# qinjr/SCoRe

Measured on AMD Instinct MI355X. Metric: train samples/sec @ batch=1024, higher is better.
Workload: dtype f32

## Files before the change

### score_amd/csrc/common.h

```cpp
#pragma once
#include <hip/hip_runtime.h>
#include <stdint.h>
#include "../../include/score_hip.h"

#define SCORE_WAVE 64

#if (defined(X3_PROBE_NOLOADA) || defined(X3_PROBE_NOLOADB) || defined(X3_PROBE_NOSPLIT) || defined(X3_PROBE_NOLDSW) ||      \
     defined(X3_PROBE_NOLDSR) || defined(X3_PROBE_NOMFMA) || defined(X3_PROBE_NOSTORE) || defined(PANEL_PROBE_NOMFMA) ||      \
     defined(PANEL_PROBE_NOALOAD) || defined(PANEL_PROBE_NOASTORE) || defined(PANEL_PROBE_NOBLOAD) ||                         \
     defined(PANEL_PROBE_NOREAD) || defined(PANEL_PROBE_NOCSTORE) || defined(GRP_NOMFMA) || defined(GRP_NOSTORE) ||           \
     defined(GRP_NOXLOAD) || defined(GSP_NOMFMA) || defined(GSP_NOBLOAD) || defined(GSP_NOSTORE) || defined(GSP_NOXLOAD) ||   \
     defined(XGP_NOMFMA) || defined(XGP_NOSTORE) || defined(XGP_NOXLOAD) || defined(AFP_NOPRELOAD) || defined(AFP_NOMFMA) ||  \
     defined(AFP_NOEPI) || defined(AFP_NOBUILD) || defined(AFP_NOTAIL) || defined(AFP_NOINP)) &&                              \
    !defined(SCORE_PROBE_BUILD)
#error "a wrong-by-design probe switch needs -DSCORE_PROBE_BUILD (tools/*_probe.py pass it; score_amd/build.py never does)"
#endif

#define SCORE_CHECK_LAUNCH()                      \
  do {                                            \
    hipError_t e__ = hipGetLastError();           \
    if (e__ != hipSuccess) return (int)e__;       \
  } while (0)

#define SCORE_TRY(expr)                           \
  do {                                            \
    int rc__ = (expr);                            \
    if (rc__ != 0) return rc__;                   \
  } while (0)

static inline int64_t cdiv64(int64_t a, int64_t b) { return (a + b - 1) / b; }
static inline int64_t align_up64(int64_t a, int64_t b) { return cdiv64(a, b) * b; }

__device__ __forceinline__ float4 ld4(const float* p) { return *reinterpret_cast<const float4*>(p); }
__device__ __forceinline__ void st4(float* p, float4 v) { *reinterpret_cast<float4*>(p) = v; }
typedef float score_v4f __attribute__((ext_vector_type(4)));
__device__ __forceinline__ float4 ld4_global(const float* p) {
  const score_v4f v = *(const __attribute__((address_space(1))) score_v4f*)p;
  return make_float4(v.x, v.y, v.z, v.w);
}
__device__ __forceinline__ float ld1_global(const float* p) { return *(const __attribute__((address_space(1))) float*)p; }
__device__ __forceinline__ float dot4(float4 a, float4 b) {
  return fmaf(a.w, b.w, fmaf(a.z, b.z, fmaf(a.y, b.y, a.x * b.x)));
}
__device__ __forceinline__ float4 fma4(float s, float4 a, float4 acc) {
  acc.x = fmaf(s, a.x, acc.x); acc.y = fmaf(s, a.y, acc.y);
  acc.z = fmaf(s, a.z, acc.z); acc.w = fmaf(s, a.w, acc.w);
  return acc;
}
__device__ __forceinline__ float4 add4(float4 a, float4 b) {
  return make_float4(a.x + b.x, a.y + b.y, a.z + b.z, a.w + b.w);
}
__device__ __forceinline__ void score_adam1(float& p, float& m, float& v, float g, float omb1, float omb2, float alpha,
                                            float eps) {
  m = __builtin_fmaf(g - m, omb1, m);
  v = __builtin_fmaf(__builtin_fmaf(g, g, -v), omb2, v);
#if defined(SCORE_ADAM_IEEE_DIV)
  p = p - (m * alpha) / (sqrtf(v) + eps);
#else
  p = p - (m * alpha) * __builtin_amdgcn_rcpf(__builtin_amdgcn_sqrtf(v) + eps);
#endif
}
__device__ __forceinline__ void score_adam_dense_body(float* __restrict__ p, float* __restrict__ m, float* __restrict__ v,
                                                      const float* __restrict__ g, int64_t n4, int64_t n, int64_t n_reg, float l2,
                                                      float alpha, float omb1, float omb2, float eps, int blk, int nblk) {
  int64_t i = (int64_t)blk * blockDim.x + threadIdx.x;
  const int64_t stride = (int64_t)nblk * blockDim.x;
  for (; i < n4; i += stride) {
    float4 mm = ld4(m + i * 4), vv = ld4(v + i * 4), gg = ld4(g + i * 4);
    int64_t e = i * 4;
    if (e >= n_reg && gg.x == 0.f && gg.y == 0.f && gg.z == 0.f && gg.w == 0.f && mm.x == 0.f && mm.y == 0.f &&
        mm.z == 0.f && mm.w == 0.f && vv.x == 0.f && vv.y == 0.f && vv.z == 0.f && vv.w == 0.f)
      continue;
    float4 pp = ld4(p + i * 4);
    if (e < n_reg) {
      gg.x = e + 0 < n_reg ? fmaf(l2, pp.x, gg.x) : gg.x;
      gg.y = e + 1 < n_reg ? fmaf(l2, pp.y, gg.y) : gg.y;
      gg.z = e + 2 < n_reg ? fmaf(l2, pp.z, gg.z) : gg.z;
      gg.w = e + 3 < n_reg ? fmaf(l2, pp.w, gg.w) : gg.w;
    }
    score_adam1(pp.x, mm.x, vv.x, gg.x, omb1, omb2, alpha, eps);
    score_adam1(pp.y, mm.y, vv.y, gg.y, omb1, omb2, alpha, eps);
    score_adam1(pp.z, mm.z, vv.z, gg.z, omb1, omb2, alpha, eps);
    score_adam1(pp.w, mm.w, vv.w, gg.w, omb1, omb2, alpha, eps);
    st4(p + i * 4, pp); st4(m + i * 4, mm); st4(v + i * 4, vv);
  }
  if (blk == 0 && threadIdx.x < (unsigned)(n - n4 * 4)) {
    int64_t e = n4 * 4 + threadIdx.x;
    float pp = p[e], mm = m[e], vv = v[e], gg = g[e];
    if (e < n_reg) gg = fmaf(l2, pp, gg);
    score_adam1(pp, mm, vv, gg, omb1, omb2, alpha, eps);
    p[e] = pp; m[e] = mm; v[e] = vv;
  }
}
__device__ __forceinline__ float sigmoidf_(float x) { return 1.0f / (1.0f + expf(-x)); }

__device__ __forceinline__ float group_sum(float v, int gs) {
  for (int off = gs >> 1; off > 0; off >>= 1) v += __shfl_xor(v, off, SCORE_WAVE);
  return v;
}
__device__ __forceinline__ float wave_sum(float v) { return group_sum(v, SCORE_WAVE); }

template <int CTRL>
__device__ __forceinline__ float dpp_f32(float v) {
  return __int_as_float(__builtin_amdgcn_update_dpp(0, __float_as_int(v), CTRL, 0xF, 0xF, true));
}
template <int N>
__device__ __forceinline__ void group_sum_n(float (&v)[N], int gs) {
  if (gs >= 2) {
#pragma unroll
    for (int n = 0; n < N; ++n) v[n] += dpp_f32<0xB1>(v[n]);
  }
  if (gs >= 4) {
#pragma unroll
    for (int n = 0; n < N; ++n) v[n] += dpp_f32<0x4E>(v[n]);
  }
  if (gs >= 8) {
#pragma unroll
    for (int n = 0; n < N; ++n) v[n] += dpp_f32<0x141>(v[n]);
  }
  if (gs >= 16) {
#pragma unroll
    for (int n = 0; n < N; ++n) v[n] += dpp_f32<0x140>(v[n]);
  }
  if (gs >= 32) {
    const int lane = (int)__builtin_amdgcn_mbcnt_hi(~0u, __builtin_amdgcn_mbcnt_lo(~0u, 0u));
    const int a16 = (lane ^ 16) << 2, a32 = (lane ^ 32) << 2;
    float t[N];
#pragma unroll
    for (int n = 0; n < N; ++n) t[n] = __int_as_float(__builtin_amdgcn_ds_bpermute(a16, __float_as_int(v[n])));
#pragma unroll
    for (int n = 0; n < N; ++n) v[n] += t[n];
    if (gs >= 64) {
#pragma unroll
      for (int n = 0; n < N; ++n) t[n] = __int_as_float(__builtin_amdgcn_ds_bpermute(a32, __float_as_int(v[n])));
#pragma unroll
      for (int n = 0; n < N; ++n) v[n] += t[n];
    }
  }
}
__device__ __forceinline__ float wave_max(float v) {
  for (int off = 32; off > 0; off >>= 1) v = fmaxf(v, __shfl_xor(v, off, SCORE_WAVE));
  return v;
}

__device__ __forceinline__ void xcd_tile_coords_n(int nwg, int orig, int gx, int gy, int& bx, int& by, int& bz) {
  const int q = nwg >> 3, r = nwg & 7, xcd = orig & 7;
  const int wg = (xcd < r ? xcd * (q + 1) : r * (q + 1) + (xcd - r) * q) + (orig >> 3);
  bx = wg % gx;
  const int t = wg / gx;
  by = t % gy;
  bz = t / gy;
}
__device__ __forceinline__ void xcd_tile_coords(int gx, int gy, int& bx, int& by, int& bz) {
  xcd_tile_coords_n((int)gridDim.x, (int)blockIdx.x, gx, gy, bx, by, bz);
}

__device__ __forceinline__ float hash_uniform(uint64_t seed, uint64_t idx) {
  uint64_t z = seed + 0x9E3779B97F4A7C15ull * (idx + 1);
  z = (z ^ (z >> 30)) * 0xBF58476D1CE4E5B9ull;
  z = (z ^ (z >> 27)) * 0x94D049BB133111EBull;
  z = z ^ (z >> 31);
  return (float)(z >> 40) * (1.0f / 16777216.0f);
}
```

### score_amd/csrc/head_fused.hip

```cpp
#include "common.h"
#include "kernels.h"

typedef float hf_f32x4 __attribute__((ext_vector_type(4)));

namespace {

constexpr int HF_ROWS = 16;
constexpr int HF_NW = 8;
constexpr int HF_CH = 16;

template <int NT>
__device__ __forceinline__ void hf_tiles(hf_f32x4 (&acc)[NT], const float* __restrict__ xs, int LD, int Kp, int K,
                                         const float* __restrict__ W, int ldw, const int (&n0)[NT], int N, int lc, int lq) {
  const int KQ = Kp >> 2;
  const int kbase = lq * KQ;
  int col[NT];
  bool cok[NT];
#pragma unroll
  for (int t = 0; t < NT; ++t) {
    cok[t] = n0[t] >= 0 && n0[t] + lc < N;
    col[t] = cok[t] ? n0[t] + lc : 0;
  }
  float b0[NT][HF_CH], b1[NT][HF_CH];
  auto fetch = [&](float (&bb)[NT][HF_CH], int s0) {
// ... 125 lines not shown
      hf_f32x4 acc[1] = {{0.f, 0.f, 0.f, 0.f}};
      const int t0 = tb + wave;
      const int n0[1] = {t0 < tend ? t0 * 16 : -1};
      if (n0[0] >= 0) hf_tiles<1>(acc, xs, LD0, Kp0, Dh, a.W1, N1, n0, N1, lc, lq);
      const int col = n0[0] + lc;
      const float bias = a.b1[min(max(col, 0), N1 - 1)];
      if (n0[0] >= 0 && col < N1) {
#pragma unroll
        for (int r = 0; r < 4; ++r) {
          const int row = b0 + lq * 4 + r;
          const float v = hf_act(acc[0][r], bias, a.drop, a.keep, a.mask0, seed0, row, col, N1);
          if (row < a.B) a.f1[(int64_t)row * N1 + col] = v;
        }
      }
    }
    return;
  }
  if (phase == 2) {
    for (int e = tid; e < HF_ROWS * N1; e += 64 * HF_NW) {
      const int i = e / N1, j = e - i * N1;
      const int row = min(b0 + i, a.B - 1);
      f1s[i * LD1 + j] = a.f1[(int64_t)row * N1 + j];
    }
  }
  for (int tb = 0; phase == 0 && tb < nt1; tb += 2 * HF_NW) {
    hf_f32x4 acc[2] = {{0.f, 0.f, 0.f, 0.f}, {0.f, 0.f, 0.f, 0.f}};
    const int t0 = tb + wave, t1 = tb + HF_NW + wave;
    const int n0[2] = {t0 < nt1 ? t0 * 16 : -1, t1 < nt1 ? t1 * 16 : -1};
    if (n0[0] >= 0) hf_tiles<2>(acc, xs, LD0, Kp0, Dh, a.W1, N1, n0, N1, lc, lq);
    float bias1[2];
#pragma unroll
    for (int t = 0; t < 2; ++t) bias1[t] = a.b1[min(max(n0[t] + lc, 0), N1 - 1)];
#pragma unroll
    for (int t = 0; t < 2; ++t) {
      const int col = n0[t] + lc;
      if (n0[t] < 0 || col >= N1) continue;
      const float bias = bias1[t];
#pragma unroll
      for (int r = 0; r < 4; ++r) {
        const int i = lq * 4 + r, row = b0 + i;
        const float v = hf_act(acc[t][r], bias, a.drop, a.keep, a.mask0, seed0, row, col, N1);
        f1s[i * LD1 + col] = v;
        if (row < a.B) a.f1[(int64_t)row * N1 + col] = v;
      }
    }
  }
  __syncthreads();

  const int nt2 = (N2 + 15) >> 4;
  for (int tb = 0; tb < nt2; tb += HF_NW) {
    hf_f32x4 acc[1] = {{0.f, 0.f, 0.f, 0.f}};
    const int t0 = tb + wave;
    const int n0[1] = {t0 < nt2 ? t0 * 16 : -1};
    if (n0[0] >= 0) hf_tiles<1>(acc, f1s, LD1, Kp1, N1, a.W2, N2, n0, N2, lc, lq);
    const int col = n0[0] + lc;
    const float bias2 = a.b2[min(max(col, 0), N2 - 1)];
    if (n0[0] >= 0 && col < N2) {
      const float bias = bias2;
#pragma unroll
      for (int r = 0; r < 4; ++r) {
        const int i = lq * 4 + r, row = b0 + i;
        const float v = hf_act(acc[0][r], bias, a.drop, a.keep, a.mask1, seed1, row, col, N2);
        f2s[i * LD2 + col] = v;
        if (row < a.B) a.f2[(int64_t)row * N2 + col] = v;
      }
    }
  }
  __syncthreads();

  if (wave == 0) {
    const int i = lane >> 2, part = lane & 3;
    float s = 0.f;
    for (int n = part; n < N2; n += 4) s = fmaf(f2s[i * LD2 + n], a.W3[n], s);
    s += __shfl_xor(s, 1, 64);
    s += __shfl_xor(s, 2, 64);
    const int row = b0 + i;
    if (part == 0 && row < a.B) {
      const float z = s + a.b3[0];
      const float p = sigmoidf_(z);
      const float lab = (float)a.label[row];
      const float eps = 1e-7f;
      a.logit[row] = z;
      a.y[row] = p;
      a.lossb[row] = -lab * logf(p + eps) - (1.0f - lab) * logf(1.0f - p + eps);
      const float dp = (-lab / (p + eps) + (1.0f - lab) / (1.0f - p + eps)) / (float)a.Bglobal;
      const float dl = dp * p * (1.0f - p);
      a.dlogit[row] = dl;
      xs[i] = dl;
    }
  }
  __syncthreads();
  if (a.dz2) {
    for (int e = tid; e < HF_ROWS * N2; e += 64 * HF_NW) {
      const int i = e / N2, n = e - i * N2, row = b0 + i;
      const float q = xs[i] * a.W3[n] / a.keep;
      if (row < a.B) a.dz2[(int64_t)row * N2 + n] = f2s[i * LD2 + n] > 0.f ? q : 0.f;
    }
  }
}


constexpr int AF_NW = 8;

struct AttnFwdArgs {
  int B, T, H, NI, N1, N2, S;
  const float* q; const float* ur; const float* ir; const float* info;
  const float* Weff; const float* qz;
  const float* W4; const float* b4; const float* w5; const float* b5; const int32_t* length;
  float* inp; float* a1; float* a2; float* score; float* head; int ldh, off_u, off_i;
  int wcopies; int64_t wstride;
};

__device__ __forceinline__ void af_build(const AttnFwdArgs& a, float* __restrict__ xs, int LD, int Kp, int row0,
                                         int row_end, int t0, int nthr) {
  const int Dk = 2 * a.H + a.NI, Dk4 = Dk >> 2, K2 = 2 * Dk;
  const int total = 16 * Dk4;
  constexpr int U = 4;
  for (int e0 = t0; e0 < total; e0 += U * nthr) {
    float4 k[U], qq[U];
    int ii[U], jj[U], gg[U];
    bool ok[U];
#pragma unroll
    for (int u = 0; u < U; ++u) {
      const int e = e0 + u * nthr;
      const int ec = e < total ? e : 0;
      ii[u] = ec / Dk4; jj[u] = (ec - ii[u] * Dk4) * 4;
      gg[u] = row0 + ii[u];
      ok[u] = e < total && gg[u] < row_end;
      const int g = gg[u] < row_end ? gg[u] : row_end - 1;
      const int j = jj[u];
      const float* src = j < a.H ? a.ur + (int64_t)g * a.H + j
                                 : (j < 2 * a.H ? a.ir + (int64_t)g * a.H + (j - a.H) : a.info + (int64_t)g * a.NI + (j - 2 * a.H));
      k[u] = ld4(src);
      qq[u] = ld4(a.q + (int64_t)(g / a.T) * Dk + j);
    }
#pragma unroll
    for (int u = 0; u < U; ++u) {
      if (e0 + u * nthr >= total) continue;
      float4 kk = k[u], qk = make_float4(qq[u].x * kk.x, qq[u].y * kk.y, qq[u].z * kk.z, qq[u].w * kk.w);
      if (ok[u]) {
#ifndef AFP_NOINP
        st4(a.inp + (int64_t)gg[u] * K2 + jj[u], kk);
        st4(a.inp + (int64_t)gg[u] * K2 + Dk + jj[u], qk);
#endif
      } else {
        kk = make_float4(0.f, 0.f, 0.f, 0.f); qk = kk;
      }
      *reinterpret_cast<float4*>(xs + ii[u] * LD + jj[u]) = kk;
      *reinterpret_cast<float4*>(xs + ii[u] * LD + Dk + jj[u]) = qk;
    }
  }
  for (int e = t0; e < 16 * (Kp - K2); e += nthr) {
    const int i = e / (Kp - K2), j = e - i * (Kp - K2);
    xs[i * LD + K2 + j] = 0.f;
  }
}

template <int KQ>
__global__ __launch_bounds__(64 * AF_NW) void attn_fwd_fused_kernel(const AttnFwdArgs a) {
  extern __shared__ float sm[];
  const int T = a.T, H = a.H, N1 = a.N1, N2 = a.N2;
  const int Dk = 2 * H + a.NI, K2 = 2 * Dk, Kp = 4 * KQ, LD = Kp + 4;
  const int L1 = N1 + 1, L2 = N2 + 1;
  float* xs0 = sm;
  float* xs1 = xs0 + 16 * LD;
  float* a1s = xs1 + 16 * LD;
  float* w4s = a1s + a.S * T * L1;
  float* a2s = w4s + N1 * N2;
  float* scs = a2s + a.S * T * L2;
  const int tid = threadIdx.x, lane = tid & 63, wave = tid >> 6;
  const int lc = lane & 15, lq = lane >> 4;
  const int b0 = blockIdx.x * a.S;
  const int ns = min(a.S, a.B - b0);
  const int row0 = b0 * T, row_end = row0 + ns * T;
  const int ntile = (ns * T + 15) >> 4;
  const int ntn = (N1 + 15) >> 4;

  float breg[KQ];
  if (wave < ntn) {
    const int col = wave * 16 + lc;
    const float* Wsrc = a.Weff + (int64_t)((blockIdx.x >> 3) % a.wcopies) * a.wstride;
#pragma unroll
    for (int s_ = 0; s_ < KQ; ++s_) {
      const int k = lq * KQ + s_;
#ifdef AFP_NOPRELOAD
      const float w = (float)(k + col) * 1e-3f;
#else
      const float w = Wsrc[(int64_t)(k < K2 ? k : K2 - 1) * N1 + (col < N1 ? col : N1 - 1)];
#endif
      breg[s_] = w * ((k < K2 && col < N1) ? 1.0f : 0.0f);
    }
  }
  for (int i = tid; i < N1 * N2; i += 64 * AF_NW) w4s[i] = a.W4[i];
  af_build(a, xs0, LD, Kp, row0, row_end, tid, 64 * AF_NW);
  __syncthreads();
  for (int m = 0; m < ntile; ++m) {
    float* xs = (m & 1) ? xs1 : xs0;
    if (wave < ntn) {
      hf_f32x4 acc[1] = {{0.f, 0.f, 0.f, 0.f}};
      const int n0[1] = {wave * 16};
      const float* xrow = xs + lc * LD + lq * KQ;
#ifndef AFP_NOMFMA
#ifdef AFP_TWOACC
      hf_f32x4 acc2 = {0.f, 0.f, 0.f, 0.f};
#pragma unroll
      for (int s4 = 0; s4 < KQ; s4 += 4) {
        const float4 av = *reinterpret_cast<const float4*>(xrow + s4);
        acc[0] = __builtin_amdgcn_mfma_f32_16x16x4f32(av.x, breg[s4 + 0], acc[0], 0, 0, 0);
        acc2 = __builtin_amdgcn_mfma_f32_16x16x4f32(av.y, breg[s4 + 1], acc2, 0, 0, 0);
        acc[0] = __builtin_amdgcn_mfma_f32_16x16x4f32(av.z, breg[s4 + 2], acc[0], 0, 0, 0);
        acc2 = __builtin_amdgcn_mfma_f32_16x16x4f32(av.w, breg[s4 + 3], acc2, 0, 0, 0);
      }
      acc[0] += acc2;
#else
#pragma unroll
      for (int s4 = 0; s4 < KQ; s4 += 4) {
        const float4 av = *reinterpret_cast<const float4*>(xrow + s4);
        acc[0] = __builtin_amdgcn_mfma_f32_16x16x4f32(av.x, breg[s4 + 0], acc[0], 0, 0, 0);
        acc[0] = __builtin_amdgcn_mfma_f32_16x16x4f32(av.y, breg[s4 + 1], acc[0], 0, 0, 0);
        acc[0] = __builtin_amdgcn_mfma_f32_16x16x4f32(av.z, breg[s4 + 2], acc[0], 0, 0, 0);
        acc[0] = __builtin_amdgcn_mfma_f32_16x16x4f32(av.w, breg[s4 + 3], acc[0], 0, 0, 0);
      }
#endif
#else
      acc[0][0] = xrow[0] * breg[0] + breg[KQ - 1];
#endif
      const int col = n0[0] + lc;
      if (col < N1) {
#pragma unroll
        for (int r = 0; r < 4; ++r) {
          const int i = m * 16 + lq * 4 + r;
          const int g = row0 + i;
          if (g < row_end) {
#ifdef AFP_NOEPI
            const float v = fmaxf(acc[0][r], 0.f);
            a1s[i * L1 + col] = v;
#else
            const float v = fmaxf(acc[0][r] + a.qz[(int64_t)(g / T) * N1 + col], 0.f);
            a1s[i * L1 + col] = v;
            a.a1[(int64_t)g * N1 + col] = v;
#endif
          }
        }
      }
    } else if (m + 1 < ntile) {
#ifndef AFP_NOBUILD
      af_build(a, (m & 1) ? xs0 : xs1, LD, Kp, row0 + (m + 1) * 16, row_end, tid - 64 * ntn, 64 * (AF_NW - ntn));
#endif
    }
    __syncthreads();
  }

#ifdef AFP_NOTAIL
  return;
#endif
  const int gsz = 64 * AF_NW / a.S, s_ = tid / gsz, gt = tid - s_ * gsz;
  const bool live = s_ < ns;
  const int b = b0 + (live ? s_ : 0);
  const float* a1b = a1s + s_ * T * L1;
  float* a2l = a2s + s_ * T * L2;
  float* sc = scs + s_ * T;
  if (live) {
    float* a2b = a.a2 + (int64_t)b * T * N2;
    for (int i = gt; i < T * N2; i += gsz) {
      const int t = i / N2, n = i - t * N2;
      float acc = 0.f;
#pragma unroll 8
      for (int k = 0; k < N1; ++k) acc = fmaf(a1b[t * L1 + k], w4s[k * N2 + n], acc);
      const float v = fmaxf(acc + a.b4[n], 0.f);
      a2l[t * L2 + n] = v;
      a2b[i] = v;
    }
  }
  __syncthreads();
  if (live) {
    const int len = a.length[b];
    for (int t = gt; t < T; t += gsz) {
      float acc = 0.f;
      for (int n = 0; n < N2; ++n) acc = fmaf(a2l[t * L2 + n], a.w5[n], acc);
      sc[t] = t < len ? acc + a.b5[0] : -4294967295.0f;
    }
  }
  __syncthreads();
  float mx = -INFINITY, den = 0.f;
  if (live) {
    for (int t = 0; t < T; ++t) mx = fmaxf(mx, sc[t]);
    for (int t = 0; t < T; ++t) den += expf(sc[t] - mx);
  }
  __syncthreads();
  if (live) {
    for (int t = gt; t < T; t += gsz) {
      const float v = expf(sc[t] - mx) / den;
      sc[t] = v;
      a.score[(int64_t)b * T + t] = v;
    }
  }
  __syncthreads();
  if (live) {
    for (int j = gt; j < 2 * H; j += gsz) {
      const bool us = j < H;
      const float* rep = (us ? a.ur : a.ir) + (int64_t)b * T * H + (us ? j : j - H);
      float acc = 0.f;
      for (int t = 0; t < T; ++t) acc = fmaf(rep[(int64_t)t * H], sc[t], acc);
      const int off = us ? a.off_u : a.off_i;
      if (off >= 0) a.head[(int64_t)b * a.ldh + off + (us ? j : j - H)] = acc;
    }
  }
}


constexpr int AB_NTW = 5;
constexpr int AB_KQ = 20;

struct AttnBwdArgs {
  int B, T, H, NI, S;
  const float* da1; const float* Weff; const float* q; const float* ur; const float* ir; const float* info;
  const float* score; const float* dhead; int ldh, off_u, off_i;
  float* dur; float* dir; float* dinfo; float* dq;
  int pool, N2;
  const float* a2; const float* a1; const float* w5; const float* W4; const int32_t* length;
  float* ds; float* da2; float* da1_out;
};

__global__ __launch_bounds__(64 * AF_NW) void attn_inp_bwd_fused_kernel(const AttnBwdArgs a) {
  extern __shared__ float sm[];
  const int T = a.T, H = a.H, NI = a.NI;
  const int Dk = 2 * H + NI, Dk4 = Dk >> 2, K2 = 2 * Dk, N1 = 4 * AB_KQ;
  const int LDA = N1 + 4, LDO = K2 + 4;
  const int RT = ((a.S * T + 15) >> 4) << 4;
  float* da1s = sm;
  float* ot = da1s + RT * LDA;
  float* dqs = ot + 16 * LDO;
  float* sds = dqs + a.S * Dk;
  float* d2s = sds + a.S * T;
  float* w4s = d2s + a.S * T * (a.N2 + 1);
  const int tid = threadIdx.x, lane = tid & 63, wave = tid >> 6;
  const int lc = lane & 15, lq = lane >> 4;
  const int b0 = blockIdx.x * a.S;
  const int ns = min(a.S, a.B - b0);
  const int row0 = b0 * T, row_end = row0 + ns * T;
  const int ntile = (ns * T + 15) >> 4;
  const int ntn = (K2 + 15) >> 4;

  float breg[AB_NTW][AB_KQ];
#pragma unroll
  for (int t = 0; t < AB_NTW; ++t) {
    const int n = (wave + AF_NW * t) * 16 + lc;
    const float msk = n < K2 ? 1.0f : 0.0f;
    const float* wrow = a.Weff + (int64_t)(n < K2 ? n : K2 - 1) * N1 + lq * AB_KQ;
#pragma unroll
    for (int s4 = 0; s4 < AB_KQ; s4 += 4) {
      const float4 w = ld4(wrow + s4);
      breg[t][s4 + 0] = w.x * msk; breg[t][s4 + 1] = w.y * msk; breg[t][s4 + 2] = w.z * msk; breg[t][s4 + 3] = w.w * msk;
    }
  }
  for (int i = tid; i < a.S * Dk; i += 64 * AF_NW) dqs[i] = 0.f;
  for (int i = tid; i < RT * LDA; i += 64 * AF_NW) da1s[i] = 0.f;
  __syncthreads();
  if (!a.pool) {
    for (int e = tid; e < ns * T * (N1 / 4); e += 64 * AF_NW) {
      const int i = e / (N1 / 4), c = (e - i * (N1 / 4)) * 4;
      *reinterpret_cast<float4*>(da1s + i * LDA + c) = ld4(a.da1 + (int64_t)(row0 + i) * N1 + c);
    }
  } else {
    const int NA = a.N2, LW = NA + 1;
    const int gsz = 64 * AF_NW / a.S, s_ = tid / gsz, gt = tid - s_ * gsz;
    const bool live = s_ < ns;
    const int b = b0 + (live ? s_ : 0);
    float* sd = sds + s_ * T;
    float* d2 = d2s + s_ * T * LW;
    for (int i = tid; i < N1 * NA; i += 64 * AF_NW) { const int k = i / NA; w4s[k * LW + (i - k * NA)] = a.W4[i]; }
    constexpr int LPT = 4;
    if (live) {
      const int gl = gt % LPT;
      const float* du = a.off_u >= 0 ? a.dhead + (int64_t)b * a.ldh + a.off_u : nullptr;
      const float* di = a.off_i >= 0 ? a.dhead + (int64_t)b * a.ldh + a.off_i : nullptr;
      for (int t0 = 0; t0 < T; t0 += gsz / LPT) {
        const int t = t0 + gt / LPT;
        const int64_t bt = (int64_t)b * T + (t < T ? t : T - 1);
        float part = 0.f;
        for (int j = gl; j < H; j += LPT) {
          if (du) part = fmaf(du[j], a.ur[bt * H + j], part);
          if (di) part = fmaf(di[j], a.ir[bt * H + j], part);
        }
        part = group_sum(part, LPT);
        if (gl == 0 && t < T) sd[t] = part;
      }
    }
    __syncthreads();
    if (live) {
      const int len = a.length[b];
      float tot = 0.f;
      for (int t = 0; t < T; ++t) tot = fmaf(a.score[(int64_t)b * T + t], sd[t], tot);
      for (int i = gt; i < T * NA; i += gsz) {
        const int t = i / NA, n = i - t * NA;
        const int64_t bt = (int64_t)b * T + t;
        const float g = t < len ? a.score[bt] * (sd[t] - tot) : 0.f;
        const float dv = a.a2[bt * NA + n] > 0.f ? g * a.w5[n] : 0.f;
        a.da2[bt * NA + n] = dv;
        d2[t * LW + n] = dv;
        if (n == 0) a.ds[bt] = g;
      }
    }
    __syncthreads();
    if (live) {
      for (int i = gt; i < T * N1; i += gsz) {
        const int t = i / N1, k = i - t * N1;
        const int64_t e = ((int64_t)b * T + t) * N1 + k;
        float acc = 0.f;
#pragma unroll 8
        for (int n = 0; n < NA; ++n) acc = fmaf(d2[t * LW + n], w4s[k * LW + n], acc);
        const float v = a.a1[e] > 0.f ? acc : 0.f;
        a.da1_out[e] = v;
        da1s[(s_ * T + t) * LDA + k] = v;
      }
    }
  }
  __syncthreads();

  for (int m = 0; m < ntile; ++m) {
    const int g0 = row0 + m * 16;
    {
      float4 av[AB_KQ / 4];
#pragma unroll
      for (int s4 = 0; s4 < AB_KQ / 4; ++s4)
        av[s4] = *reinterpret_cast<const float4*>(da1s + (m * 16 + lc) * LDA + lq * AB_KQ + 4 * s4);
#pragma unroll
      for (int t = 0; t < AB_NTW; ++t) {
        const int n0 = (wave + AF_NW * t) * 16;
        if (n0 >= ntn * 16) continue;
        hf_f32x4 acc = {0.f, 0.f, 0.f, 0.f};
#pragma unroll
        for (int s4 = 0; s4 < AB_KQ / 4; ++s4) {
          acc = __builtin_amdgcn_mfma_f32_16x16x4f32(av[s4].x, breg[t][4 * s4 + 0], acc, 0, 0, 0);
          acc = __builtin_amdgcn_mfma_f32_16x16x4f32(av[s4].y, breg[t][4 * s4 + 1], acc, 0, 0, 0);
          acc = __builtin_amdgcn_mfma_f32_16x16x4f32(av[s4].z, breg[t][4 * s4 + 2], acc, 0, 0, 0);
          acc = __builtin_amdgcn_mfma_f32_16x16x4f32(av[s4].w, breg[t][4 * s4 + 3], acc, 0, 0, 0);
        }
        const int col = n0 + lc;
        if (col < K2) {
#pragma unroll
          for (int r = 0; r < 4; ++r) ot[(lq * 4 + r) * LDO + col] = acc[r];
        }
      }
    }
    __syncthreads();
    constexpr int U = 3;
    for (int e0 = tid; e0 < 16 * Dk4; e0 += U * 64 * AF_NW) {
      float4 kv[U], qq[U], pl[U];
      float sc[U];
      int ii[U], jj[U], gg[U];
      bool ok[U];
#pragma unroll
      for (int u = 0; u < U; ++u) {
        const int e = e0 + u * 64 * AF_NW;
        const int ec = e < 16 * Dk4 ? e : 0;
        ii[u] = ec / Dk4; jj[u] = (ec - ii[u] * Dk4) * 4;
        gg[u] = g0 + ii[u];
        ok[u] = e < 16 * Dk4 && gg[u] < row_end;
        const int g = gg[u] < row_end ? gg[u] : row_end - 1;
        const int j = jj[u], b = g / T;
        const float* src = j < H ? a.ur + (int64_t)g * H + j : (j < 2 * H ? a.ir + (int64_t)g * H + (j - H) : a.info + (int64_t)g * NI + (j - 2 * H));
        kv[u] = ld4(src);
        qq[u] = ld4(a.q + (int64_t)b * Dk + j);
        sc[u] = a.score[g];
        const int off = j < H ? a.off_u : a.off_i;
        const bool hasp = j < 2 * H && off >= 0;
        const float4 p4 = ld4(a.dhead + (int64_t)b * a.ldh + (hasp ? off + (j < H ? j : j - H) : 0));
        const float pm = hasp ? 1.0f : 0.0f;
        pl[u] = make_float4(p4.x * pm, p4.y * pm, p4.z * pm, p4.w * pm);
      }
#pragma unroll
      for (int u = 0; u < U; ++u) {
        if (e0 + u * 64 * AF_NW >= 16 * Dk4) continue;
        float* o1 = ot + ii[u] * LDO + jj[u];
        const float4 d1 = *reinterpret_cast<const float4*>(o1);
        const float4 d3 = *reinterpret_cast<const float4*>(o1 + Dk);
        float4 pr = make_float4(0.f, 0.f, 0.f, 0.f);
        if (ok[u]) {
          const int j = jj[u];
          float4 o;
          o.x = fmaf(d3.x, qq[u].x, d1.x) + pl[u].x * sc[u]; o.y = fmaf(d3.y, qq[u].y, d1.y) + pl[u].y * sc[u];
          o.z = fmaf(d3.z, qq[u].z, d1.z) + pl[u].z * sc[u]; o.w = fmaf(d3.w, qq[u].w, d1.w) + pl[u].w * sc[u];
          float* dst = j < H ? a.dur + (int64_t)gg[u] * H + j
                             : (j < 2 * H ? a.dir + (int64_t)gg[u] * H + (j - H) : a.dinfo + (int64_t)gg[u] * NI + (j - 2 * H));
          st4(dst, o);
          pr = make_float4(d3.x * kv[u].x, d3.y * kv[u].y, d3.z * kv[u].z, d3.w * kv[u].w);
        }
        *reinterpret_cast<float4*>(o1) = pr;
      }
    }
    __syncthreads();
    for (int e = tid; e < ns * Dk4; e += 64 * AF_NW) {
      const int s_ = e / Dk4, j = (e - s_ * Dk4) * 4;
      const int lo = max(0, s_ * T - m * 16), hi = min(16, (s_ + 1) * T - m * 16);
      if (lo < hi) {
        float4 acc = *reinterpret_cast<const float4*>(dqs + s_ * Dk + j);
        for (int i = lo; i < hi; ++i) {
          const float4 v = *reinterpret_cast<const float4*>(ot + i * LDO + j);
          acc.x += v.x; acc.y += v.y; acc.z += v.z; acc.w += v.w;
        }
        *reinterpret_cast<float4*>(dqs + s_ * Dk + j) = acc;
      }
    }
    __syncthreads();
  }
  for (int e = tid; e < ns * Dk4; e += 64 * AF_NW) {
    const int s_ = e / Dk4, j = (e - s_ * Dk4) * 4;
    st4(a.dq + (int64_t)(b0 + s_) * Dk + j, *reinterpret_cast<const float4*>(dqs + s_ * Dk + j));
  }
}


constexpr int HB_K2Q = 20;
constexpr int HB_K1Q = 52;

struct HeadBwdArgs {
  int B, Dh;
  const float* dz2; const float* W2; const float* f1; float keep;
  const float* W1; const float* x; const float* gamma; float rs;
  float* dz1; float* dbn; float* dhead; float* tmp;
};

__global__ __launch_bounds__(64 * HF_NW) void head_bwd_fused_kernel(const HeadBwdArgs a) {
  constexpr int N1 = 4 * HB_K2Q * 0 + 200, N2 = 80, KP1 = 4 * HB_K1Q;
  constexpr int LD2 = N2 + 4, LD1 = KP1 + 4;
  __shared__ __attribute__((aligned(16))) float z2s[HF_ROWS * LD2];
  __shared__ __attribute__((aligned(16))) float z1s[HF_ROWS * LD1];
  const int tid = threadIdx.x, lane = tid & 63, wave = tid >> 6;
  const int lc = lane & 15, lq = lane >> 4;
  const int b0 = blockIdx.x * HF_ROWS;
  for (int e = tid; e < HF_ROWS * (N2 / 4); e += 64 * HF_NW) {
    const int i = e / (N2 / 4), c = (e - i * (N2 / 4)) * 4;
    const int row = b0 + i < a.B ? b0 + i : a.B - 1;
    float4 v = ld4(a.dz2 + (int64_t)row * N2 + c);
    if (b0 + i >= a.B) v = make_float4(0.f, 0.f, 0.f, 0.f);
    *reinterpret_cast<float4*>(z2s + i * LD2 + c) = v;
  }
  for (int e = tid; e < HF_ROWS * (LD1 - N1); e += 64 * HF_NW) {
    const int i = e / (LD1 - N1), c = e - i * (LD1 - N1);
    z1s[i * LD1 + N1 + c] = 0.f;
  }
  float b2[2][HB_K2Q];
#pragma unroll
  for (int t = 0; t < 2; ++t) {
    const int n = (wave + HF_NW * t) * 16 + lc;
    const float msk = n < N1 ? 1.0f : 0.0f;
    const float* wrow = a.W2 + (int64_t)(n < N1 ? n : N1 - 1) * N2 + lq * HB_K2Q;
#pragma unroll
    for (int s4 = 0; s4 < HB_K2Q; s4 += 4) {
      const float4 w = ld4(wrow + s4);
      b2[t][s4 + 0] = w.x * msk; b2[t][s4 + 1] = w.y * msk; b2[t][s4 + 2] = w.z * msk; b2[t][s4 + 3] = w.w * msk;
    }
  }
  __syncthreads();
  {
    float4 av[HB_K2Q / 4];
#pragma unroll
    for (int s4 = 0; s4 < HB_K2Q / 4; ++s4) av[s4] = *reinterpret_cast<const float4*>(z2s + lc * LD2 + lq * HB_K2Q + 4 * s4);
#pragma unroll
    for (int t = 0; t < 2; ++t) {
      const int n0 = (wave + HF_NW * t) * 16;
      if (n0 >= N1) continue;
      hf_f32x4 acc = {0.f, 0.f, 0.f, 0.f};
#pragma unroll
      for (int s4 = 0; s4 < HB_K2Q / 4; ++s4) {
        acc = __builtin_amdgcn_mfma_f32_16x16x4f32(av[s4].x, b2[t][4 * s4 + 0], acc, 0, 0, 0);
        acc = __builtin_amdgcn_mfma_f32_16x16x4f32(av[s4].y, b2[t][4 * s4 + 1], acc, 0, 0, 0);
        acc = __builtin_amdgcn_mfma_f32_16x16x4f32(av[s4].z, b2[t][4 * s4 + 2], acc, 0, 0, 0);
        acc = __builtin_amdgcn_mfma_f32_16x16x4f32(av[s4].w, b2[t][4 * s4 + 3], acc, 0, 0, 0);
      }
      const int col = n0 + lc;
      if (col < N1) {
        float y[4];
#pragma unroll
        for (int r = 0; r < 4; ++r) y[r] = a.f1[(int64_t)min(b0 + lq * 4 + r, a.B - 1) * N1 + col];
#pragma unroll
        for (int r = 0; r < 4; ++r) {
          const int i = lq * 4 + r, row = b0 + i;
          const float q = acc[r] / a.keep;
          const float v = (row < a.B && y[r] > 0.f) ? q : 0.f;
          if (row < a.B && blockIdx.y == 0) a.dz1[(int64_t)row * N1 + col] = v;
          z1s[i * LD1 + col] = v;
        }
      }
    }
  }
  __syncthreads();
  const int nt_all = (a.Dh + 15) >> 4;
  const int per = (nt_all + (int)gridDim.y - 1) / (int)gridDim.y;
  const int t0 = (int)blockIdx.y * per, nt = min(nt_all, t0 + per);
  float4 av[HB_K1Q / 4];
#pragma unroll
  for (int s4 = 0; s4 < HB_K1Q / 4; ++s4) av[s4] = *reinterpret_cast<const float4*>(z1s + lc * LD1 + lq * HB_K1Q + 4 * s4);
  float4 bw[2][HB_K1Q / 4];
  auto fetch = [&](float4 (&dst)[HB_K1Q / 4], int tile) {
    const int n = tile * 16 + lc;
    const float* wrow = a.W1 + (int64_t)(n < a.Dh ? n : a.Dh - 1) * N1 + lq * HB_K1Q;
#pragma unroll
    for (int s4 = 0; s4 < HB_K1Q / 4; ++s4) {
      const int k = lq * HB_K1Q + 4 * s4;
      dst[s4] = ld4(k + 3 < N1 ? wrow + 4 * s4 : a.W1);
    }
  };
  if (t0 + wave < nt) fetch(bw[0], t0 + wave);
  int cur = 0;
  for (int tile = t0 + wave; tile < nt; tile += HF_NW, cur ^= 1) {
    if (tile + HF_NW < nt) {
      if (cur == 0) fetch(bw[1], tile + HF_NW); else fetch(bw[0], tile + HF_NW);
    }
    hf_f32x4 acc = {0.f, 0.f, 0.f, 0.f};
    const int col = tile * 16 + lc;
    const float cm = col < a.Dh ? 1.0f : 0.0f;
#pragma unroll
    for (int s4 = 0; s4 < HB_K1Q / 4; ++s4) {
      const float4 w = cur == 0 ? bw[0][s4] : bw[1][s4];
      acc = __builtin_amdgcn_mfma_f32_16x16x4f32(av[s4].x, w.x * cm, acc, 0, 0, 0);
      acc = __builtin_amdgcn_mfma_f32_16x16x4f32(av[s4].y, w.y * cm, acc, 0, 0, 0);
      acc = __builtin_amdgcn_mfma_f32_16x16x4f32(av[s4].z, w.z * cm, acc, 0, 0, 0);
      acc = __builtin_amdgcn_mfma_f32_16x16x4f32(av[s4].w, w.w * cm, acc, 0, 0, 0);
    }
    {
      const int cc = col < a.Dh ? col : a.Dh - 1;
      const float gs = a.gamma[cc] * a.rs;
      float xv[4];
#pragma unroll
      for (int r = 0; r < 4; ++r) xv[r] = a.x[(int64_t)min(b0 + lq * 4 + r, a.B - 1) * a.Dh + cc];
#pragma unroll
      for (int r = 0; r < 4; ++r) {
        const int row = b0 + lq * 4 + r;
        if (row < a.B && col < a.Dh) {
          const int64_t e = (int64_t)row * a.Dh + col;
          const float dy = acc[r];
          a.dbn[e] = dy;
          a.dhead[e] = dy * gs;
          a.tmp[e] = dy * (xv[r] * a.rs);
        }
      }
    }
  }
}

}

bool score_head_fwd_fused_fits(int B, int Dh, int N1, int N2) {
  const int LD0 = ((Dh + 15) & ~15) + 4, LD1 = ((N1 + 15) & ~15) + 4, LD2 = ((N2 + 15) & ~15) + 4;
  return B > 0 && (size_t)HF_ROWS * (LD0 + LD1 + LD2) * sizeof(float) <= 150 * 1024;
}

int score_launch_head_fwd_fused(int B, int Dh, int N1, int N2, const float* x, const float* gamma, const float* beta,
                                float rs, const float* W1, const float* b1, const float* W2, const float* b2,
                                const float* W3, const float* b3, float keep, const uint8_t* mask0, const uint8_t* mask1,
                                uint64_t seed0, uint64_t seed1, const int32_t* label, float* bn, float* f1, float* f2,
                                float* logit, float* y, float* lossb, float* dlogit, int Bglobal, hipStream_t s,
                                const uint64_t* seed_dev, float* dz2, int single_launch) {
  const int LD0 = ((Dh + 15) & ~15) + 4, LD1 = ((N1 + 15) & ~15) + 4, LD2 = ((N2 + 15) & ~15) + 4;
  const size_t lds = (size_t)HF_ROWS * (LD0 + LD1 + LD2) * sizeof(float);
  if (!score_head_fwd_fused_fits(B, Dh, N1, N2)) return SCORE_E_SHAPE;
  static thread_local bool attr_set = false;
  if (!attr_set && lds > 48 * 1024) {
    hipError_t e = hipFuncSetAttribute(reinterpret_cast<const void*>(head_fwd_fused_kernel),
                                       hipFuncAttributeMaxDynamicSharedMemorySize, 150 * 1024);
    if (e != hipSuccess) return (int)e;
    attr_set = true;
  }
  HeadFwdArgs a;
  a.B = B; a.Dh = Dh; a.N1 = N1; a.N2 = N2; a.Bglobal = Bglobal;
  a.x = x; a.gamma = gamma; a.beta = beta; a.rs = rs;
  a.W1 = W1; a.b1 = b1; a.W2 = W2; a.b2 = b2; a.W3 = W3; a.b3 = b3;
  a.keep = keep; a.drop = keep < 1.f ? 1 : 0; a.mask0 = mask0; a.mask1 = mask1; a.seed0 = seed0; a.seed1 = seed1; a.seed_dev = seed_dev;
  a.label = label; a.bn = bn; a.f1 = f1; a.f2 = f2; a.logit = logit; a.y = y; a.lossb = lossb; a.dlogit = dlogit;
  a.dz2 = dz2;
  const int mt = (B + HF_ROWS - 1) / HF_ROWS, nt1 = (N1 + 15) >> 4;
  const bool split = !single_launch && nt1 >= 4 && mt >= 32;
  if (!split) {
    a.phase = 0;
    hipLaunchKernelGGL(head_fwd_fused_kernel, dim3(mt), dim3(64 * HF_NW), lds, s, a);
    SCORE_CHECK_LAUNCH();
    return 0;
  }
  a.phase = 1;
  hipLaunchKernelGGL(head_fwd_fused_kernel, dim3(mt, 4), dim3(64 * HF_NW), lds, s, a);
  SCORE_CHECK_LAUNCH();
  a.phase = 2;
  hipLaunchKernelGGL(head_fwd_fused_kernel, dim3(mt), dim3(64 * HF_NW), lds, s, a);
  SCORE_CHECK_LAUNCH();
  return 0;
}

int score_launch_attn_fwd_fused(int B, int T, int H, int NI, int N1, int N2, const float* q, const float* ur,
                                const float* ir, const float* info, const float* Weff, const float* qz, const float* W4,
                                const float* b4, const float* w5, const float* b5, const int32_t* length, float* inp,
                                float* a1, float* a2, float* score, float* head, int ldh, int off_u, int off_i,
                                hipStream_t s, int weff_copies, int64_t weff_copy_stride) {
  if (B <= 0 || T <= 0 || (H & 3) || (NI & 3) || N1 > 16 * 5 || N1 <= 0 || N2 <= 0 || (int64_t)B * T >= (1LL << 30))
    return SCORE_E_SHAPE;
  const int K2 = 2 * (2 * H + NI), Kp = (K2 + 15) & ~15, LD = Kp + 4;
  int S = B >= 4 * 256 ? 4 : B >= 2 * 256 ? 2 : 1;
  size_t lds = 0;
  for (; S >= 1; S >>= 1) {
    lds = ((size_t)2 * 16 * LD + (size_t)S * T * (N1 + 1) + (size_t)N1 * N2 + (size_t)S * T * (N2 + 1) + (size_t)S * T) * sizeof(float);
    if (lds <= 150 * 1024) break;
  }
  if (S < 1) return SCORE_E_SHAPE;
  const int kq = Kp / 4;
  if (kq != 148 && kq != 52 && kq != 44 && kq != 36 && kq != 84) return SCORE_E_SHAPE;
  static thread_local bool attr_set = false;
  if (!attr_set) {
    for (const void* f : {reinterpret_cast<const void*>(attn_fwd_fused_kernel<148>),
                          reinterpret_cast<const void*>(attn_fwd_fused_kernel<52>),
                          reinterpret_cast<const void*>(attn_fwd_fused_kernel<44>),
                          reinterpret_cast<const void*>(attn_fwd_fused_kernel<36>),
                          reinterpret_cast<const void*>(attn_fwd_fused_kernel<84>)}) {
      hipError_t e = hipFuncSetAttribute(f, hipFuncAttributeMaxDynamicSharedMemorySize, 150 * 1024);
      if (e != hipSuccess) return (int)e;
    }
    attr_set = true;
  }
  AttnFwdArgs a;
  a.B = B; a.T = T; a.H = H; a.NI = NI; a.N1 = N1; a.N2 = N2; a.S = S;
  a.q = q; a.ur = ur; a.ir = ir; a.info = info; a.Weff = Weff; a.qz = qz;
  a.W4 = W4; a.b4 = b4; a.w5 = w5; a.b5 = b5; a.length = length;
  a.inp = inp; a.a1 = a1; a.a2 = a2; a.score = score; a.head = head; a.ldh = ldh; a.off_u = off_u; a.off_i = off_i;
  a.wcopies = weff_copies > 0 ? weff_copies : 1; a.wstride = weff_copy_stride;
  const dim3 grid((B + S - 1) / S), block(64 * AF_NW);
  switch (Kp / 4) {
    case 148: hipLaunchKernelGGL(attn_fwd_fused_kernel<148>, grid, block, lds, s, a); break;
    case 52: hipLaunchKernelGGL(attn_fwd_fused_kernel<52>, grid, block, lds, s, a); break;
    case 44: hipLaunchKernelGGL(attn_fwd_fused_kernel<44>, grid, block, lds, s, a); break;
    case 36: hipLaunchKernelGGL(attn_fwd_fused_kernel<36>, grid, block, lds, s, a); break;
    case 84: hipLaunchKernelGGL(attn_fwd_fused_kernel<84>, grid, block, lds, s, a); break;
    default: return SCORE_E_SHAPE;
  }
  SCORE_CHECK_LAUNCH();
  return 0;
}

static bool ab_plan(int B, int T, int H, int NI, int N1, int N2, int ldh, int off_u, int off_i, bool pool, int* S_out,
                    size_t* lds_out) {
  const int Dk = 2 * H + NI, K2 = 2 * Dk;
  if (B <= 0 || T <= 0 || (H & 3) || (NI & 3) || N1 != 4 * AB_KQ || K2 > 16 * AF_NW * AB_NTW || (int64_t)B * T >= (1LL << 30) ||
      (ldh & 3) || (off_u >= 0 && (off_u & 3)) || (off_i >= 0 && (off_i & 3)) || (pool && N2 <= 0))
    return false;
  const int S = B >= 4 * 256 ? 4 : B >= 2 * 256 ? 2 : 1;
  const int RT = ((S * T + 15) >> 4) << 4;
  const size_t lds = ((size_t)RT * (N1 + 4) + (size_t)16 * (K2 + 4) + (size_t)S * Dk +
                      (pool ? (size_t)S * T + (size_t)S * T * (N2 + 1) + (size_t)N1 * (N2 + 1) : 0)) * sizeof(float);
  if (lds > 150 * 1024) return false;
  *S_out = S; *lds_out = lds;
  return true;
}
bool score_attn_inp_bwd_fused_fits(int B, int T, int H, int NI, int N1, int N2, int ldh, int off_u, int off_i, bool pool) {
  int S; size_t lds;
  return ab_plan(B, T, H, NI, N1, N2, ldh, off_u, off_i, pool, &S, &lds);
}

int score_launch_attn_inp_bwd_fused(int B, int T, int H, int NI, int N1, const float* da1, const float* Weff, const float* q,
                                    const float* ur, const float* ir, const float* info, const float* score,
                                    const float* dhead, int ldh, int off_u, int off_i, float* dur, float* dir, float* dinfo,
                                    float* dq, hipStream_t s, int N2, const float* a2, const float* a1, const float* w5,
                                    const float* W4, const int32_t* length, float* ds, float* da2, float* da1_out) {
  const int pool = a2 != nullptr;
  if (pool && (!a1 || !w5 || !W4 || !length || !ds || !da2 || !da1_out)) return SCORE_E_BADARG;
  int S; size_t lds;
  if (!ab_plan(B, T, H, NI, N1, N2, ldh, off_u, off_i, pool != 0, &S, &lds)) return SCORE_E_SHAPE;
  static thread_local bool attr_set = false;
  if (!attr_set) {
    hipError_t e = hipFuncSetAttribute(reinterpret_cast<const void*>(attn_inp_bwd_fused_kernel),
                                       hipFuncAttributeMaxDynamicSharedMemorySize, 150 * 1024);
    if (e != hipSuccess) return (int)e;
    attr_set = true;
  }
  AttnBwdArgs a;
  a.B = B; a.T = T; a.H = H; a.NI = NI; a.S = S;
  a.da1 = da1; a.Weff = Weff; a.q = q; a.ur = ur; a.ir = ir; a.info = info; a.score = score; a.dhead = dhead;
  a.ldh = ldh; a.off_u = off_u; a.off_i = off_i; a.dur = dur; a.dir = dir; a.dinfo = dinfo; a.dq = dq;
  a.pool = pool; a.N2 = pool ? N2 : 0; a.a2 = a2; a.a1 = a1; a.w5 = w5; a.W4 = W4; a.length = length; a.ds = ds; a.da2 = da2;
  a.da1_out = da1_out;
  hipLaunchKernelGGL(attn_inp_bwd_fused_kernel, dim3((B + S - 1) / S), dim3(64 * AF_NW), lds, s, a);
  SCORE_CHECK_LAUNCH();
  return 0;
}

int score_launch_head_bwd_fused(int B, int Dh, int N1, int N2, const float* dz2, const float* W2, const float* f1, float keep,
                                const float* W1, const float* x, const float* gamma, float rs, float* dz1, float* dbn,
                                float* dhead, float* tmp, hipStream_t s) {
  if (B <= 0 || Dh <= 0 || N1 != 200 || N2 != 80) return SCORE_E_SHAPE;
  HeadBwdArgs a;
  a.B = B; a.Dh = Dh; a.dz2 = dz2; a.W2 = W2; a.f1 = f1; a.keep = keep; a.W1 = W1; a.x = x; a.gamma = gamma; a.rs = rs;
  a.dz1 = dz1; a.dbn = dbn; a.dhead = dhead; a.tmp = tmp;
  const int mt = (B + HF_ROWS - 1) / HF_ROWS, ntile = (Dh + 15) >> 4;
  const int ny = (mt <= 128 && ntile >= 4 * HF_NW) ? (mt <= 64 ? 4 : 2) : 1;
  hipLaunchKernelGGL(head_bwd_fused_kernel, dim3(mt, ny), dim3(64 * HF_NW), 0, s, a);
  SCORE_CHECK_LAUNCH();
  return 0;
}
```

Measured before the change: 915,100.

## Add specialized large-K attention forward kernel with register-resident weights

Adds a new attn_fwd_large_kernel for the K2≈600 case (KS=19) at large batch. It holds the Weff slice in registers per wave and splits K across waves, then reduces partial MFMA results through LDS. It also software-pipelines the next tile's global loads behind the current MFMA and unrolls the final weighted-sum over T. The intent is to remove repeated weight loads from LDS or global memory and to hide input-load latency. In exchange it raises register pressure and adds a cross-wave LDS reduction and extra synchronisation.

```diff
diff --git a/score_amd/csrc/common.h b/score_amd/csrc/common.h
--- a/score_amd/csrc/common.h
+++ b/score_amd/csrc/common.h
@@ -11,7 +11,7 @@
      defined(PANEL_PROBE_NOREAD) || defined(PANEL_PROBE_NOCSTORE) || defined(GRP_NOMFMA) || defined(GRP_NOSTORE) ||           \
      defined(GRP_NOXLOAD) || defined(GSP_NOMFMA) || defined(GSP_NOBLOAD) || defined(GSP_NOSTORE) || defined(GSP_NOXLOAD) ||   \
      defined(XGP_NOMFMA) || defined(XGP_NOSTORE) || defined(XGP_NOXLOAD) || defined(AFP_NOPRELOAD) || defined(AFP_NOMFMA) ||  \
-     defined(AFP_NOEPI) || defined(AFP_NOBUILD) || defined(AFP_NOTAIL) || defined(AFP_NOINP)) &&                              \
+     defined(AFP_NOEPI) || defined(AFP_NOBUILD) || defined(AFP_NOTAIL) || defined(AFP_NOINP) || defined(AFP_NOLARGE)) &&      \
     !defined(SCORE_PROBE_BUILD)
 #error "a wrong-by-design probe switch needs -DSCORE_PROBE_BUILD (tools/*_probe.py pass it; score_amd/build.py never does)"
 #endif
diff --git a/score_amd/csrc/head_fused.hip b/score_amd/csrc/head_fused.hip
--- a/score_amd/csrc/head_fused.hip
+++ b/score_amd/csrc/head_fused.hip
@@ -451,6 +451,232 @@
       const float* rep = (us ? a.ur : a.ir) + (int64_t)b * T * H + (us ? j : j - H);
       float acc = 0.f;
       for (int t = 0; t < T; ++t) acc = fmaf(rep[(int64_t)t * H], sc[t], acc);
+      const int off = us ? a.off_u : a.off_i;
+      if (off >= 0) a.head[(int64_t)b * a.ldh + off + (us ? j : j - H)] = acc;
+    }
+  }
+}
+
+
+constexpr int AL_S = 4;
+constexpr int AL_RL = 84;
+constexpr int AL_TB = 6;
+constexpr int AL_K4 = 20;
+
+template <int KS>
+__global__ __launch_bounds__(64 * AF_NW) void attn_fwd_large_kernel(const AttnFwdArgs a) {
+  extern __shared__ float sm[];
+  constexpr int Kp = 32 * KS, LD = Kp + 4;
+  constexpr int U = (16 * (Kp / 8) + 64 * AF_NW - 1) / (64 * AF_NW);
+  constexpr int NTH = 64 * AF_NW;
+  const int T = a.T, H = a.H, N1 = a.N1, N2 = a.N2;
+  const int Dk = 2 * H + a.NI, Dk4 = Dk >> 2, K2 = 2 * Dk;
+  const int L1 = N1 + 1, L2 = N2 + 1;
+  float* xs = sm;
+  float* red = xs + 16 * LD;
+  float* a1s = red + AF_NW * 16 * AL_RL;
+  float* w4s = a1s + AL_S * T * L1;
+  float* a2s = w4s + N1 * N2;
+  float* scs = a2s + AL_S * T * L2;
+  const int tid = threadIdx.x, lane = tid & 63, wave = tid >> 6;
+  const int lc = lane & 15, lq = lane >> 4;
+  const int b0 = blockIdx.x * AL_S;
+  const int ns = min(AL_S, a.B - b0);
+  const int row0 = b0 * T, row_end = row0 + ns * T;
+  const int ntile = (ns * T + 15) >> 4;
+  const int total = 16 * Dk4;
+
+  float4 kreg[U], qreg[U];
+  auto request = [&](int m) {
+#pragma unroll
+    for (int u = 0; u < U; ++u) {
+      const int e = tid + u * NTH;
+      const int ec = e < total ? e : 0;
+      const int i = ec / Dk4, j = (ec - i * Dk4) * 4;
+      const int g = min(row0 + m * 16 + i, row_end - 1);
+      const float* src = j < H ? a.ur + (int64_t)g * H + j
+                               : (j < 2 * H ? a.ir + (int64_t)g * H + (j - H) : a.info + (int64_t)g * a.NI + (j - 2 * H));
+      kreg[u] = ld4(src);
+      qreg[u] = ld4(a.q + (int64_t)(g / T) * Dk + j);
+    }
+  };
+  auto deposit = [&](int m) {
+#pragma unroll
+    for (int u = 0; u < U; ++u) {
+      const int e = tid + u * NTH;
+      if (e >= total) continue;
+      const int i = e / Dk4, j = (e - i * Dk4) * 4;
+      const int g = row0 + m * 16 + i;
+      float4 kk = kreg[u], qk = make_float4(qreg[u].x * kk.x, qreg[u].y * kk.y, qreg[u].z * kk.z, qreg[u].w * kk.w);
+      if (g < row_end) {
+#ifndef AFP_NOINP
+        st4(a.inp + (int64_t)g * K2 + j, kk);
+        st4(a.inp + (int64_t)g * K2 + Dk + j, qk);
+#endif
+      } else {
+        kk = make_float4(0.f, 0.f, 0.f, 0.f); qk = kk;
+      }
+      *reinterpret_cast<float4*>(xs + i * LD + j) = kk;
+      *reinterpret_cast<float4*>(xs + i * LD + Dk + j) = qk;
+    }
+  };
+
+  request(0);
+  const int kw = wave * 4 * KS + lq * KS;
+  float breg[5][KS];
+  {
+    const float* Wsrc = a.Weff + (int64_t)((blockIdx.x >> 3) % a.wcopies) * a.wstride;
+#pragma unroll
+    for (int s_ = 0; s_ < KS; ++s_) {
+      const int k = kw + s_;
+#pragma unroll
+      for (int t = 0; t < 5; ++t) {
+        const int col = t * 16 + lc;
+#ifdef AFP_NOPRELOAD
+        const float w = (float)(k + col) * 1e-3f;
+#else
+        const float w = Wsrc[(int64_t)(k < K2 ? k : K2 - 1) * N1 + (col < N1 ? col : N1 - 1)];
+#endif
+        breg[t][s_] = w * ((k < K2 && col < N1) ? 1.0f : 0.0f);
+      }
+    }
+  }
+  for (int i = tid; i < N1 * N2; i += NTH) w4s[i] = a.W4[i];
+  for (int e = tid; e < 16 * (LD - K2); e += NTH) {
+    const int i = e / (LD - K2), j = e - i * (LD - K2);
+    xs[i * LD + K2 + j] = 0.f;
+  }
+  deposit(0);
+  __syncthreads();
+  for (int m = 0; m < ntile; ++m) {
+    if (m + 1 < ntile) request(m + 1);
+    constexpr int UE = (16 * 80 + NTH - 1) / NTH;
+    float qzv[UE];
+#pragma unroll
+    for (int u = 0; u < UE; ++u) {
+      const int e = min(tid + u * NTH, 16 * N1 - 1);
+      const int i = e / N1, col = e - i * N1;
+      qzv[u] = a.qz[(int64_t)(min(row0 + m * 16 + i, row_end - 1) / T) * N1 + col];
+    }
+    {
+      hf_f32x4 acc[5];
+#pragma unroll
+      for (int t = 0; t < 5; ++t) acc[t] = hf_f32x4{0.f, 0.f, 0.f, 0.f};
+      const float* xrow = xs + lc * LD + kw;
+#ifndef AFP_NOMFMA
+#pragma unroll
+      for (int s_ = 0; s_ < KS; ++s_) {
+        const float av = xrow[s_];
+#pragma unroll
+        for (int t = 0; t < 5; ++t) acc[t] = __builtin_amdgcn_mfma_f32_16x16x4f32(av, breg[t][s_], acc[t], 0, 0, 0);
+      }
+#else
+#pragma unroll
+      for (int t = 0; t < 5; ++t) acc[t][0] = xrow[t] * breg[t][0] + breg[t][KS - 1];
+#endif
+      float* rw = red + wave * 16 * AL_RL;
+#pragma unroll
+      for (int t = 0; t < 5; ++t)
+#pragma unroll
+        for (int r = 0; r < 4; ++r) rw[(lq * 4 + r) * AL_RL + t * 16 + lc] = acc[t][r];
+    }
+    __syncthreads();
+    if (m + 1 < ntile) deposit(m + 1);
+#pragma unroll
+    for (int u = 0; u < UE; ++u) {
+      const int e = tid + u * NTH;
+      if (e >= 16 * N1) continue;
+      const int i = e / N1, col = e - i * N1;
+      const int g = row0 + m * 16 + i;
+      float v = red[i * AL_RL + col];
+#pragma unroll
+      for (int w = 1; w < AF_NW; ++w) v += red[w * 16 * AL_RL + i * AL_RL + col];
+      if (g < row_end) {
+        v = fmaxf(v + qzv[u], 0.f);
+        a1s[(m * 16 + i) * L1 + col] = v;
+        a.a1[(int64_t)g * N1 + col] = v;
+      }
+    }
+    __syncthreads();
+  }
+
+#ifdef AFP_NOTAIL
+  return;
+#endif
+  const int nrow = ns * T;
+  {
+    const int ntn2 = (N2 + 15) >> 4;
+    for (int job = wave; job < ntile * ntn2; job += AF_NW) {
+      const int mt = job / ntn2, nt = job - mt * ntn2;
+      const int col = nt * 16 + lc, colc = min(col, N2 - 1);
+      const int arow = mt * 16 + lc;
+      const float* ar = a1s + min(arow, nrow - 1) * L1;
+      const float am = arow < nrow ? 1.0f : 0.0f;
+      hf_f32x4 acc = {0.f, 0.f, 0.f, 0.f};
+#pragma unroll
+      for (int k4 = 0; k4 < AL_K4; ++k4) {
+        const int k = lq * AL_K4 + k4, kc = min(k, N1 - 1);
+        const float bm = (k < N1 && col < N2) ? 1.0f : 0.0f;
+        acc = __builtin_amdgcn_mfma_f32_16x16x4f32(ar[kc] * am, w4s[kc * N2 + colc] * bm, acc, 0, 0, 0);
+      }
+      const float bias = a.b4[colc];
+#pragma unroll
+      for (int r = 0; r < 4; ++r) {
+        const int row = mt * 16 + lq * 4 + r;
+        if (row < nrow && col < N2) {
+          const float v = fmaxf(acc[r] + bias, 0.f);
+          a2s[row * L2 + col] = v;
+          a.a2[(int64_t)(row0 + row) * N2 + col] = v;
+        }
+      }
+    }
+  }
+  __syncthreads();
+  for (int r0 = 0; r0 < nrow; r0 += NTH / 4) {
+    const int row = r0 + (tid >> 2), part = tid & 3;
+    const int rc = min(row, nrow - 1);
+    float acc = 0.f;
+    for (int n = part; n < N2; n += 4) acc = fmaf(a2s[rc * L2 + n], a.w5[n], acc);
+    acc += __shfl_xor(acc, 1, 64);
+    acc += __shfl_xor(acc, 2, 64);
+    if (part == 0 && row < nrow) {
+      const int sb = row / T, t = row - sb * T;
+      scs[row] = t < a.length[b0 + sb] ? acc + a.b5[0] : -4294967295.0f;
+    }
+  }
+  __syncthreads();
+  constexpr int gsz = NTH / AL_S;
+  const int s_ = tid / gsz, gt = tid - s_ * gsz;
+  const bool live = s_ < ns;
+  const int b = b0 + (live ? s_ : 0);
+  float* sc = scs + s_ * T;
+  float mx = -INFINITY, den = 0.f;
+  if (live) {
+    for (int t = 0; t < T; ++t) mx = fmaxf(mx, sc[t]);
+    for (int t = 0; t < T; ++t) den += expf(sc[t] - mx);
+  }
+  __syncthreads();
+  if (live) {
+    for (int t = gt; t < T; t += gsz) {
+      const float v = expf(sc[t] - mx) / den;
+      sc[t] = v;
+      a.score[(int64_t)b * T + t] = v;
+    }
+  }
+  __syncthreads();
+  if (live) {
+    for (int j = gt; j < 2 * H; j += gsz) {
+      const bool us = j < H;
+      const float* rep = (us ? a.ur : a.ir) + (int64_t)b * T * H + (us ? j : j - H);
+      float acc = 0.f;
+      for (int t0 = 0; t0 < T; t0 += AL_TB) {
+        float rv[AL_TB];
+#pragma unroll
+        for (int u = 0; u < AL_TB; ++u) rv[u] = rep[(int64_t)min(t0 + u, T - 1) * H];
+#pragma unroll
+        for (int u = 0; u < AL_TB; ++u)
+          if (t0 + u < T) acc = fmaf(rv[u], sc[t0 + u], acc);
+      }
       const int off = us ? a.off_u : a.off_i;
       if (off >= 0) a.head[(int64_t)b * a.ldh + off + (us ? j : j - H)] = acc;
     }
@@ -845,6 +1071,32 @@
   if (B <= 0 || T <= 0 || (H & 3) || (NI & 3) || N1 > 16 * 5 || N1 <= 0 || N2 <= 0 || (int64_t)B * T >= (1LL << 30))
     return SCORE_E_SHAPE;
   const int K2 = 2 * (2 * H + NI), Kp = (K2 + 15) & ~15, LD = Kp + 4;
+  AttnFwdArgs a;
+  a.B = B; a.T = T; a.H = H; a.NI = NI; a.N1 = N1; a.N2 = N2;
+  a.q = q; a.ur = ur; a.ir = ir; a.info = info; a.Weff = Weff; a.qz = qz;
+  a.W4 = W4; a.b4 = b4; a.w5 = w5; a.b5 = b5; a.length = length;
+  a.inp = inp; a.a1 = a1; a.a2 = a2; a.score = score; a.head = head; a.ldh = ldh; a.off_u = off_u; a.off_i = off_i;
+  a.wcopies = weff_copies > 0 ? weff_copies : 1; a.wstride = weff_copy_stride;
+#ifndef AFP_NOLARGE
+  constexpr int KSL = 19;
+  if (B >= 4 * 256 && (K2 + 31) / 32 == KSL && N1 <= 4 * AL_K4) {
+    const size_t ldl = ((size_t)16 * (32 * KSL + 4) + (size_t)AF_NW * 16 * AL_RL + (size_t)AL_S * T * (N1 + 1) + (size_t)N1 * N2 +
+                        (size_t)AL_S * T * (N2 + 1) + (size_t)AL_S * T) * sizeof(float);
+    if (ldl <= 150 * 1024) {
+      static thread_local bool large_attr_set = false;
+      if (!large_attr_set) {
+        hipError_t e = hipFuncSetAttribute(reinterpret_cast<const void*>(attn_fwd_large_kernel<KSL>),
+                                           hipFuncAttributeMaxDynamicSharedMemorySize, 150 * 1024);
+        if (e != hipSuccess) return (int)e;
+        large_attr_set = true;
+      }
+      a.S = AL_S;
+      hipLaunchKernelGGL(attn_fwd_large_kernel<KSL>, dim3((B + AL_S - 1) / AL_S), dim3(64 * AF_NW), ldl, s, a);
+      SCORE_CHECK_LAUNCH();
+      return 0;
+    }
+  }
+#endif
   int S = B >= 4 * 256 ? 4 : B >= 2 * 256 ? 2 : 1;
   size_t lds = 0;
   for (; S >= 1; S >>= 1) {
@@ -866,12 +1118,7 @@
     }
     attr_set = true;
   }
-  AttnFwdArgs a;
-  a.B = B; a.T = T; a.H = H; a.NI = NI; a.N1 = N1; a.N2 = N2; a.S = S;
-  a.q = q; a.ur = ur; a.ir = ir; a.info = info; a.Weff = Weff; a.qz = qz;
-  a.W4 = W4; a.b4 = b4; a.w5 = w5; a.b5 = b5; a.length = length;
-  a.inp = inp; a.a1 = a1; a.a2 = a2; a.score = score; a.head = head; a.ldh = ldh; a.off_u = off_u; a.off_i = off_i;
-  a.wcopies = weff_copies > 0 ? weff_copies : 1; a.wstride = weff_copy_stride;
+  a.S = S;
   const dim3 grid((B + S - 1) / S), block(64 * AF_NW);
   switch (Kp / 4) {
     case 148: hipLaunchKernelGGL(attn_fwd_fused_kernel<148>, grid, block, lds, s, a); break;
```

New measurement: 866,700 (median of 2 runs). 5.3% lower.
